# raguilar011095/planet_heightmap_generation

Measured on AMD Instinct MI355X. Metric: Mcells·iter/s, terrain-post erosion stack, higher is better.
Workload: dtype f64

## Files before the change

### planet_heightmap_generation_amd/csrc/device.h

```cpp
#pragma once
#include <hip/hip_runtime.h>

#include <cstdint>
#include <cstdio>
#include <map>
#include <string>
#include <vector>

#include "device_mem.h"
#include "host_util.h"

#include "erode_ops.h"
#include "flood_ops.h"
#include "wo_internal.h"

namespace wo {

#define WO_TRY try {
#define WO_CATCH(fn)                                                                                   \
    } catch (const ::wo::HipError& e) { ::wo::set_error(std::string(fn) + ": " + e.msg); return 2; }   \
      catch (const std::exception& e) { ::wo::set_error(std::string(fn) + ": " + e.what()); return 3; }

constexpr int WO_BLOCK = 256;
inline int blocks_for(int64_t n, int maxBlocks = 1 << 20) {
// ... 82 lines not shown
    wo::FloodExchange floodX;
    void* floodLink = nullptr; void (*floodLinkFree)(void*) = nullptr;
    wo_flood_gpu fgpu;

    int32_t *d_off = nullptr, *d_adj = nullptr;
    float *d_dist = nullptr, *d_xyz = nullptr;
    float *d_e = nullptr, *d_e2 = nullptr, *d_hot = nullptr, *d_orig = nullptr;
    uint8_t *d_ocean = nullptr, *d_coast = nullptr;
    int64_t mirrorMaskVersion = -1;
    uint8_t* d_oceanKnown = nullptr; int32_t* d_maskDiff = nullptr; bool oceanKnownValid = false;
    bool hot_valid = false;
    float* d_savedE = nullptr; uint8_t* d_savedOcean = nullptr; bool saved = false;
    uint8_t* d_tables = nullptr;
    bool scratch = false;
    bool landIdentity = false;
    int64_t floodPrefixMirror = -1, floodPrefixStatic = -1;
    bool floodPrefixOk = false;
    int32_t *d_landIdx = nullptr, *d_land[2] = {nullptr, nullptr}, *d_rank = nullptr;
    int32_t* d_landInit = nullptr; int64_t oceanVersion = 0, landListsOcean = -1; bool landListsMirror = false; int32_t landListsL = -1;
    uint32_t* d_keys[2] = {nullptr, nullptr};
    float *d_cellDist = nullptr, *d_flow = nullptr;
    wo::SolveTask* d_task = nullptr; wo::SolveOut* d_out = nullptr;
    int32_t *d_haloSend = nullptr, *d_haloRecv = nullptr; float *d_haloBuf = nullptr, *h_haloBuf = nullptr; int32_t nHaloSend = 0, nHaloRecv = 0;
    int32_t* d_flowCnt = nullptr; wo::TargetRank* d_tr = nullptr; wo::EventList* d_ev = nullptr; float* d_me = nullptr;
    int32_t *d_carveSlot = nullptr, *d_carveDeps = nullptr, *d_carveDepCnt = nullptr, *d_carveDepPos = nullptr;
    uint32_t* d_rs[2] = {nullptr, nullptr}; int rsFlip[2] = {0, 0};
    wo::CarveRec* d_carveRecs = nullptr; wo::CarveExpect* d_carveExpect = nullptr; unsigned long long* d_carveG = nullptr;
    int32_t* d_carveSlotDone = nullptr; int64_t carveCap = 0;
    unsigned long long* d_accCnt = nullptr;
    int32_t *d_ftLr = nullptr, *d_ftParent = nullptr, *d_ftExtCnt = nullptr; uint32_t* d_ftInflow = nullptr; unsigned long long* d_ftRootAcc = nullptr;
    int32_t *d_jump = nullptr, *d_nj = nullptr;
    int32_t* d_doneAt = nullptr;
    double* d_totalExcess = nullptr;
    float *d_glac = nullptr, *d_iceFlow = nullptr;
    int32_t *d_iceTarget = nullptr, *d_arank = nullptr;
    uint8_t* d_iceUp = nullptr;
    int32_t *d_patchOrder = nullptr, *d_slotOf = nullptr, *d_patchPending = nullptr, *d_patchTotals = nullptr, *d_patchBlk = nullptr;
    int64_t patchVersion = -1; bool patchMirror = false; int32_t numPatches = 0; int64_t lastPatchLaunches = 1; int64_t solveCalls = 0;
    hipStream_t side = nullptr; hipEvent_t evFork = nullptr, evJoin = nullptr; bool onSide = false;
    uint32_t* d_basinKey = nullptr; int32_t* d_basinVals[2] = {nullptr, nullptr}; int32_t *d_basinJ = nullptr, *d_basinSlot = nullptr, *d_basinRange = nullptr;
    uint8_t* d_basinLong = nullptr; int64_t basinLaunches = 0;
    wo::Affine* d_affine[2] = {nullptr, nullptr};
    int64_t solvePassSerial = 0;
    int32_t* h_patchTotals = nullptr;
    int32_t *d_listA = nullptr, *d_listB = nullptr, *d_counters = nullptr;
    void* d_sortTemp = nullptr; size_t sortTempBytes = 0;
    int landCur = 0;
    int32_t L = 0;

    struct Import {
        wo::DeviceArena mem;
        uint8_t* img = nullptr; int64_t imgCap = 0;
        int32_t* label = nullptr;
        uint8_t* flags = nullptr;
        int32_t* lists = nullptr;
        uint8_t* seedOcean = nullptr;
        int32_t* blockCounts = nullptr;
        int32_t* totals = nullptr; int32_t* h_totals = nullptr;
    } imp;

    struct wo_wind_block* wind = nullptr;
    struct wo_ocean_block* ocean = nullptr;
    struct wo_precip_block* precip = nullptr;
    struct wo_temp_block* temp = nullptr;
    struct wo_koppen_block* koppen = nullptr;
    struct wo_map_block* map = nullptr;
// ... 91 lines not shown
```

### planet_heightmap_generation_amd/csrc/erode_ops.h

```cpp
#pragma once
#include <cmath>
#include <cstdint>
#include <cstring>

#include "noise.h"

namespace wo {

constexpr int WO_MAX_DEG = 24;
constexpr int32_t WO_NOT_DONE = 0x7fffffff;

#ifndef WO_TASK_ALIGN
#define WO_TASK_ALIGN 16
#endif
struct alignas(WO_TASK_ALIGN) SolveTask {
    int32_t predSelf, predT, predT2;
    uint32_t flags;
    float e0r, e0t, e0t2;
    float cellDistT;
    double factor;
    int32_t pad_[2];
};
static_assert(sizeof(SolveTask) == 48, "one 48-byte record per task");
#ifndef WO_PATCH_CELLS
// ... 18 lines not shown
    const int32_t* off;
    const int32_t* adj;
    const float* dist;
    const float* xyz;
    const uint8_t* ocean;
    const uint8_t* coast;
    float* e;
    float* e2;
    float* me;
    int32_t L;
    int32_t* land;
    const int32_t* landIdx;
    int32_t xcdTileL;
    int32_t* rank;
    int32_t* target;
    TargetRank* tr;
    float* cellDist;
    float* flow;
    uint32_t* accA; uint32_t* accB;
    unsigned long long* accCnt;
    int32_t* jumpA; int32_t* jumpB;
    SolveTask* task;
    const int32_t* slotOf;
    SolveOut* out;
    double solveK, solveM, solveDt;
    int32_t solveFinals;
    int32_t solveLean;
    int32_t* basinJ;
    const int32_t* basinMslot;
    int32_t* blk;
    EventList* ev;
    int32_t* doneAt;
    double* totalExcess;
    float* glac;
    int32_t* iceTarget;
    float* iceFlow;
    uint8_t* iceUp;
    int32_t* arank;
    const int32_t* carveSlot;
    int32_t* carveDeps;
    int32_t* carveDepCnt;
    int32_t* carveDepPos;
    int32_t* blocker;
};

WO_HD inline double nd_or_eps(float d) { return (d == 0.0f || d != d) ? 1e-6 : (double)d; }

constexpr int WO_ROW = 8;
struct alignas(4) RowI4 { int32_t v[4]; };
struct alignas(4) RowF4 { float v[4]; };
WO_HD inline int load_row(const Fields& F, int32_t r, int32_t& b, int32_t (&nb)[WO_ROW]) {
    b = F.off[r];
    const int deg = F.off[r + 1] - b;
#if defined(__HIP_DEVICE_COMPILE__)
    static_assert(WO_ROW == 8, "two RowI4 per row");
    const RowI4 lo = *reinterpret_cast<const RowI4*>(F.adj + b), hi = *reinterpret_cast<const RowI4*>(F.adj + b + 4);
#pragma unroll
    for (int k = 0; k < 4; ++k) { nb[k] = (k < deg) ? lo.v[k] : r; nb[k + 4] = (k + 4 < deg) ? hi.v[k] : r; }
#else
#pragma unroll
    for (int k = 0; k < WO_ROW; ++k) nb[k] = (k < deg) ? F.adj[b + k] : r;
#endif
    return deg;
}
WO_HD inline void load_row_dist(const Fields& F, int32_t b, int deg, float (&dd)[WO_ROW]) {
#if defined(__HIP_DEVICE_COMPILE__)
// ... 476 lines not shown
#pragma unroll
        for (int k = 0; k < WO_ROW; ++k) if (k < deg && q[k].target == x && q[k].rank < bestRank) { best = nbs[k]; bestRank = q[k].rank; }
    } else {
        for (int32_t j = b; j < b + deg; ++j) {
            const int32_t n = F.adj[j];
            const TargetRank v = F.tr[n];
            if (v.target != x) continue;
            if (v.rank < bestRank) { best = n; bestRank = v.rank; }
        }
    }
    return best;
}
WO_HD inline float solve_final_cell(const Fields& F, int32_t x) {
    if (F.ocean[x]) return F.e[x];
    if (F.ev) {
        const EventList E = F.ev[x];
        if (E.rank[0] != -2) {
            int32_t last = -1;
#pragma unroll
            for (int q = 0; q < WO_EVENTS; ++q) if (E.rank[q] >= 0) last = E.cell[q];
            if (last < 0) return F.e[x];
            return (last == x) ? F.out[store_index(F, x)].self.v : F.out[store_index(F, last)].dep.v;
        }
    }
    const int32_t best = latest_event_cell(F, x);
    if (best < 0) return F.e[x];
    return (best == x) ? F.out[store_index(F, x)].self.v : F.out[store_index(F, best)].dep.v;
}

WO_HD inline float masked_elev_cell(const Fields& F, int32_t r) { return F.ocean[r] ? INFINITY : F.e[r]; }

WO_HD inline bool talus_may_exceed(double x, double d, double talus) { return x > talus * d * (1.0 - 1e-12); }

template <class Masked>
WO_HD inline void thermal_excess_cell_t(const Fields& F, int32_t r, double talus, Masked masked) {
    double total = 0;
    if (!F.ocean[r]) {
        const double h = masked(r);
        int32_t b, nbs[WO_ROW];
        const int deg = load_row(F, r, b, nbs);
        if (deg <= WO_ROW) {
            float mh[WO_ROW], dd[WO_ROW];
#pragma unroll
            for (int k = 0; k < WO_ROW; ++k) mh[k] = masked(nbs[k]);
            load_row_dist(F, b, deg, dd);
#pragma unroll
            for (int k = 0; k < WO_ROW; ++k) {
                const double nh = mh[k];
                if (k >= deg || nh >= h) continue;
                const double d = nd_or_eps(dd[k]);
                if (!talus_may_exceed(h - nh, d, talus)) continue;
                const double slope = (h - nh) / d;
                if (slope > talus) total += (slope - talus) * d;
            }
        } else {
            for (int32_t j = b; j < b + deg; ++j) {
                const double nh = masked(F.adj[j]);
                if (nh >= h) continue;
                const double d = nd_or_eps(F.dist[j]);
                const double slope = (h - nh) / d;
                if (slope > talus) total += (slope - talus) * d;
            }
        }
    }
    F.totalExcess[r] = total;
}

WO_HD inline void thermal_excess_cell(const Fields& F, int32_t r, double talus) { thermal_excess_cell_t(F, r, talus, [&](int32_t c) { return F.me[c]; }); }

template <class Masked>
WO_HD inline float thermal_apply_row(const Fields& F, double h, int32_t myRank, double myTotal, int32_t b, const int32_t (&nbs)[WO_ROW], int deg,
                                     double talus, double kThermal, Masked masked) {
    float mh[WO_ROW], dd[WO_ROW];
#pragma unroll
    for (int k = 0; k < WO_ROW; ++k) mh[k] = masked(nbs[k]);
    load_row_dist(F, b, deg, dd);
    double inSh[WO_ROW], outSh[WO_ROW]; int32_t inRk[WO_ROW]; bool outOn[WO_ROW];
    bool hasOut = false, hasIn = false;
#pragma unroll
    for (int k = 0; k < WO_ROW; ++k) {
        inRk[k] = 0x7fffffff; inSh[k] = 0; outSh[k] = 0; outOn[k] = false;
        const double nh = mh[k], d = nd_or_eps(dd[k]);
        const double gap = fabs(nh - h);
        if (!(k < deg && nh != (double)INFINITY && talus_may_exceed(gap, d, talus))) continue;
        const double slope = gap / d;
        if (!(slope > talus)) continue;
        const bool sends = nh < h;
        if (!sends && !(nh > h)) continue;
// ... 65 lines not shown
    if (nIn == 0 && !hasOut) return (float)(h + 0.0);
    float delta = 0.0f;
    int32_t last = -1;
    for (int phase = 0; phase < 2; ++phase) {
        for (;;) {
            int pick = -1; int32_t pr = 0x7fffffff;
            for (int k = 0; k < nIn; ++k) { const int32_t rk = inRank[k * stride]; if (rk > last && rk < pr) { pr = rk; pick = k; } }
            if (pick < 0 || (phase == 0 && pr > myRank)) break;
            delta = (float)((double)delta + inShare[pick * stride]);
            last = pr;
        }
        if (phase == 0 && hasOut && outShare) {
            for (int k = 0; k < nOut; ++k) delta = (float)((double)delta - outShare[k * stride]);
        } else if (phase == 0 && hasOut) {
            for (int32_t j = b; j < b + deg; ++j) {
                const double nh = (double)F.me[F.adj[j]];
                if (!(nh < h)) continue;
                const double d = nd_or_eps(F.dist[j]);
                const double slope = (h - nh) / d;
                if (slope > talus) {
                    const float excess = (float)((slope - talus) * d);
                    delta = (float)((double)delta - ((double)excess / myTotal) * myTransfer);
                }
            }
        }
    }
    return (float)(h + (double)delta);
}

WO_HD inline float thermal_apply_cell(const Fields& F, int32_t c, double talus, double kThermal, double* inShare, int32_t* inRank, int stride,
                                      double* outShare = nullptr) {
    return thermal_apply_cell_t(F, c, talus, kThermal, inShare, inRank, stride, outShare, [&](int32_t x) { return F.me[x]; });
}

WO_HD inline double smoothstep_js(double x, double e0, double e1) {
    double t = (x - e0) / (e1 - e0);
    if (!(t < 1)) t = (t != t) ? t : 1;
    if (!(t > 0)) t = (t != t) ? t : 0;
    return t * t * (3 - 2 * t);
}

WO_HD inline float glac_index_cell(const Fields& F, int32_t r, double glacialStrength) {
    if (F.ocean[r]) return 0.0f;
    const double PI_ = 3.141592653589793;
    const double thresholdLat = PI_ / 2 - glacialStrength * PI_ / 4.5;
    double y = F.xyz[3 * r + 1];
    if (y > 1) y = 1;
    if (y < -1) y = -1;
    const double polarDist = fabs(asin(y));
    const double latFactor = smoothstep_js(polarDist, thresholdLat, PI_ / 2);
    const double elevFactor = smoothstep_js(F.e[r], 0.5, 0.9);
    const double latScale = smoothstep_js(polarDist, PI_ / 8, PI_ / 3);
    const double a = latFactor, b = elevFactor * 0.3 * (0.3 + 0.7 * latScale);
    return (float)((a > b ? a : b) * glacialStrength);
}

WO_HD inline void ice_receiver_cell(const Fields& F, int32_t r) {
    int32_t bestNb = -1;
    if (!F.ocean[r] && F.glac[r] > 0) {
        const double h = F.e[r];
        double bestDrop = 0;
        for (int32_t j = F.off[r]; j < F.off[r + 1]; ++j) {
            const int32_t nb = F.adj[j];
            const double drop = h - (double)F.e[nb];
            if (drop > bestDrop) { bestDrop = drop; bestNb = nb; }
        }
// ... 243 lines not shown
```

### planet_heightmap_generation_amd/csrc/kernels_impl.h

```cpp
#pragma once
#include <hip/hip_runtime.h>
#include <hip/hip_cooperative_groups.h>

#include "device.h"
#include "plates_ops.h"
#include "climate_ops.h"

namespace wo {

#define WO_GRID_STRIDE(i, n) for (int32_t i = blockIdx.x * blockDim.x + threadIdx.x; i < (n); i += gridDim.x * blockDim.x)

#define WO_XCD_CELLS(r, n)                                                                                           \
    for (int32_t xi_ = (int32_t)(blockIdx.x >> 3), xt_ = F.xcdTile,                                                  \
                 r = (int32_t)((((xi_ / xt_) * 8 + (int32_t)(blockIdx.x & 7u)) * xt_ + (xi_ % xt_)) * (int32_t)blockDim.x + (int32_t)threadIdx.x), \
                 once_ = 1;                                                                                          \
         once_ && r < (n); once_ = 0)

#define WO_XCD_LAND(i, r)                                                                                            \
    for (int32_t xi_ = (int32_t)(blockIdx.x >> 3), xt_ = F.xcdTileL,                                                 \
                 i = (int32_t)((((xi_ / xt_) * 8 + (int32_t)(blockIdx.x & 7u)) * xt_ + (xi_ % xt_)) * (int32_t)blockDim.x + (int32_t)threadIdx.x), \
                 once_ = 1;                                                                                          \
         once_ && i < F.L; once_ = 0)                                                                                \
        for (int32_t r = F.landIdx ? F.landIdx[i] : i, once2_ = 1; once2_; once2_ = 0)

// ... 127 lines not shown
        F.jumpA[r] = -1; F.flow[r] = 0.0f; F.totalExcess[r] = 0.0; F.me[r] = INFINITY;
    }
}
constexpr int WO_TILE_WIN = 4096;
constexpr int WO_TILE_MARGIN = 256;
struct TileWindow {
    const float* g; const float* s; int32_t lo, hi;
    __device__ inline float operator()(int32_t c) const { return (c >= lo && c <= hi) ? s[c - lo] : g[c]; }
};
__device__ inline TileWindow stage_tile(const Fields& F, const float* field, float* s_buf, int32_t i0) {
    TileWindow W; W.g = field; W.s = s_buf; W.lo = 1; W.hi = 0;
    if (!F.tileLds) return W;
    if (i0 < F.L) {
        const int32_t i1 = min(i0 + (int32_t)blockDim.x, F.L) - 1;
        const int32_t lo = max((F.landIdx ? F.landIdx[i0] : i0) - WO_TILE_MARGIN, 0), hi = min((F.landIdx ? F.landIdx[i1] : i1) + WO_TILE_MARGIN, F.N - 1);
        if (hi - lo + 1 <= WO_TILE_WIN) {
            for (int32_t k = threadIdx.x; k <= hi - lo; k += blockDim.x) s_buf[k] = field[lo + k];
            W.lo = lo; W.hi = hi;
        }
    }
    __syncthreads();
    return W;
}
#define WO_XCD_LAND_BASE() ((int32_t)(((((int32_t)(blockIdx.x >> 3) / F.xcdTileL) * 8 + (int32_t)(blockIdx.x & 7u)) * F.xcdTileL + ((int32_t)(blockIdx.x >> 3) % F.xcdTileL)) * (int32_t)blockDim.x))

__global__ __launch_bounds__(WO_BLOCK) void k_receivers_flow_init(Fields F, int32_t* donorCnt) {
    __shared__ float s_tile[WO_TILE_WIN];
    const TileWindow E = stage_tile(F, F.e, s_tile, WO_XCD_LAND_BASE());
    WO_XCD_LAND(i, r) {
        const int32_t t = receiver_cell_t(F, r, E);
        int32_t j = -1; const uint32_t a = 1;
        if (t >= 0 && !F.ocean[t] && F.rank[r] < F.rank[t]) j = t;
        if (F.accA) F.accA[r] = a;
        F.jumpA[r] = j; F.accCnt[r] = 1ull;
        if (j >= 0 && donorCnt) atomicAdd(&donorCnt[j], 1);
        if (F.basinJ) {
            const bool landT = t >= 0 && !F.ocean[t];
            const int32_t sr = F.basinMslot ? F.basinMslot[r] : r;
            F.basinJ[sr] = landT ? (F.basinMslot ? F.basinMslot[t] : t) : sr;
        }
    }
}
__global__ __launch_bounds__(WO_BLOCK) void k_flow_climb(Fields F, const int32_t* donorCnt, int32_t cap) {
    WO_XCD_LAND(i, r) {
        int32_t d = r;
        if (!(donorCnt[d] == 0 && F.jumpA[d] >= 0)) continue;
        unsigned long long v = 1;
        int32_t j = F.jumpA[d];
        for (int32_t step = 0; step < cap; ++step) {
            const int32_t donors = donorCnt[j];
            const int32_t jj = F.jumpA[j];
            const unsigned long long old = atomicAdd(&F.accCnt[j], (1ull << 32) | v);
            F.jumpA[d] = -2;
            if ((int32_t)(old >> 32) + 1 != donors) break;
            if (jj < 0) break;
            d = j;
            j = jj;
            v = (old & 0xffffffffull) + v;
        }
    }
}
#ifndef WO_FT_CELLS
#define WO_FT_CELLS 1024
#endif
#ifndef WO_FT_THREADS
#define WO_FT_THREADS 256
#endif
constexpr int FT_CELLS = WO_FT_CELLS, FT_THREADS = WO_FT_THREADS, FT_PER = FT_CELLS / FT_THREADS;
static_assert(FT_CELLS % FT_THREADS == 0 && FT_CELLS < 0xffff, "tile cells are 16-bit indices");
struct FlowTiles {
    int32_t* lr;
    unsigned long long* rootAcc;
    uint32_t* inflow;
    int32_t* extCnt;
    int32_t* parent;
    int32_t* basinJ;
};
template <bool FINAL>
__global__ __launch_bounds__(FT_THREADS) void k_flow_tiles(Fields F, FlowTiles T) {
    __shared__ uint32_t s_pc[FT_CELLS];
    __shared__ unsigned long long s_acc[FT_CELLS];
    __shared__ uint16_t s_lr[FINAL ? 1 : FT_CELLS];
    __shared__ uint16_t s_b[FINAL ? 1 : FT_CELLS];
    __shared__ int32_t s_bext[FINAL ? 1 : FT_CELLS];
    const int tid = threadIdx.x;
    const int32_t base = (int32_t)blockIdx.x * FT_CELLS;
    const int32_t n = min((int32_t)FT_CELLS, F.L - base);
#pragma unroll
    for (int q = 0; q < FT_PER; ++q) {
        const int i = tid + q * FT_THREADS;
        if (i >= n) continue;
        const int32_t j = F.jumpA[base + i];
        const bool local = j >= base && j < base + n;
        s_pc[i] = local ? (uint32_t)(j - base) : 0xffffu;
        uint32_t w = 1u;
        if (FINAL) { w += T.inflow[base + i]; T.inflow[base + i] = 0u; T.extCnt[base + i] = 0; }
        s_acc[i] = (unsigned long long)w;
        if (!FINAL) s_lr[i] = local ? (uint16_t)(j - base) : (uint16_t)i;
        if (!FINAL && T.basinJ) {
            const int32_t jb = T.basinJ[base + i];
            s_b[i] = (jb >= base && jb < base + n) ? (uint16_t)(jb - base) : (uint16_t)i;
            s_bext[i] = jb;
        }
    }
    __syncthreads();
#pragma unroll
    for (int q = 0; q < FT_PER; ++q) {
        const int i = tid + q * FT_THREADS;
        if (i >= n) continue;
        const uint32_t p = s_pc[i] & 0xffffu;
        if (p != 0xffffu) atomicAdd(&s_pc[p], 1u << 16);
    }
    __syncthreads();
#pragma unroll
    for (int q = 0; q < FT_PER; ++q) {
        const int i = tid + q * FT_THREADS;
        if (i >= n) continue;
        const uint32_t pc0 = s_pc[i];
        if ((pc0 >> 16) != 0u || (pc0 & 0xffffu) == 0xffffu) continue;
        uint32_t p = pc0 & 0xffffu;
        uint32_t v = (uint32_t)s_acc[i];
        for (;;) {
            const uint32_t pcp = s_pc[p];
            const unsigned long long old = atomicAdd(&s_acc[p], (1ull << 32) | (unsigned long long)v);
            if ((uint32_t)(old >> 32) + 1u != (pcp >> 16)) break;
            v += (uint32_t)old;
            p = pcp & 0xffffu;
            if (p == 0xffffu) break;
        }
    }
    __syncthreads();
#pragma unroll
    for (int q = 0; q < FT_PER; ++q) {
        const int i = tid + q * FT_THREADS;
        if (i >= n) continue;
        const uint32_t total = (uint32_t)s_acc[i];
        if (FINAL) F.accCnt[base + i] = (unsigned long long)total;
        else {
            uint16_t r = s_lr[i];
            for (int it = 0; it < FT_CELLS; ++it) {
                const uint16_t rr = s_lr[r];
                if (rr == r) break;
                s_lr[i] = rr;
                r = rr;
            }
            T.lr[base + i] = base + (int32_t)r;
            if ((s_pc[i] & 0xffffu) == 0xffffu) T.rootAcc[base + i] = (unsigned long long)total;
            if (T.basinJ) {
                const uint16_t b0 = s_b[r];
                int32_t out = s_bext[r];
                if (b0 != r) {
                    int32_t res = -1;
                    uint16_t c = b0;
                    for (int it = 0; it < 64; ++it) {
                        const uint16_t cc = s_b[c];
                        if (cc == c) { res = s_bext[c]; break; }
                        if (cc == r) break;
                        c = cc;
                    }
                    out = res >= 0 ? res : ((uint16_t)i == r ? s_bext[i] : base + (int32_t)r);
                }
                T.basinJ[base + i] = out;
            }
        }
    }
}
__global__ __launch_bounds__(WO_BLOCK) void k_flow_root_links(Fields F, FlowTiles T) {
    WO_GRID_STRIDE(i, F.L) {
        if (T.lr[i] != i) continue;
        const int32_t x = F.jumpA[i];
        int32_t P = -1;
        if (x >= 0) { P = T.lr[x]; atomicAdd(&T.extCnt[P], 1); }
        T.parent[i] = P;
    }
}
__global__ __launch_bounds__(WO_BLOCK) void k_flow_root_climb(Fields F, FlowTiles T) {
    WO_GRID_STRIDE(i, F.L) {
        if (T.lr[i] != i || T.extCnt[i] != 0) continue;
        int32_t P = T.parent[i];
        if (P < 0) continue;
        int32_t x = F.jumpA[i];
        uint32_t v = (uint32_t)T.rootAcc[i];
        for (;;) {
            const int32_t need = T.extCnt[P];
            const int32_t PP = T.parent[P];
            const int32_t xx = F.jumpA[P];
            atomicAdd(&T.inflow[x], v);
            const unsigned long long old = atomicAdd(&T.rootAcc[P], (1ull << 32) | (unsigned long long)v);
            if ((int32_t)(old >> 32) + 1 != need) break;
            if (PP < 0) break;
            v += (uint32_t)old;
            P = PP; x = xx;
        }
    }
}

// ... 263 lines not shown
}

__global__ __launch_bounds__(WO_BLOCK) void k_solve_blk_init(Fields F, int32_t L) {
    WO_GRID_STRIDE(s, L) {
        if (F.out[s].self.tag != 0) continue;
        const SolveTask T = F.task[s];
        F.blk[s] = T.predT >= 0 ? T.predT : (T.predSelf >= 0 ? T.predSelf : T.predT2);
    }
}
__global__ __launch_bounds__(WO_BLOCK) void k_slot_scatter(const int32_t* patchOrder, int32_t* slotOf, int32_t L) {
    WO_GRID_STRIDE(s, L) slotOf[patchOrder[s]] = s;
}


__global__ __launch_bounds__(WO_BLOCK) void k_solve_final(Fields F, float* out, float* masked) {
    WO_XCD_LAND(i, r) {
        const float v = solve_final_cell(F, r);
        out[r] = v;
        if (masked) masked[r] = v;
    }
}
__global__ __launch_bounds__(WO_BLOCK) void k_fill_i32(int32_t* a, int32_t v, int32_t n) { WO_GRID_STRIDE(i, n) a[i] = v; }

__global__ __launch_bounds__(WO_BLOCK) void k_masked_elev(Fields F) { WO_XCD_LAND(i, r) F.me[r] = F.e[r]; }
__global__ __launch_bounds__(WO_BLOCK) void k_thermal_excess(Fields F, double talus) {
    __shared__ float s_tile[WO_TILE_WIN];
    const TileWindow M = stage_tile(F, F.me, s_tile, WO_XCD_LAND_BASE());
    WO_XCD_LAND(i, r) thermal_excess_cell_t(F, r, talus, M);
}
#ifndef WO_THERMAL_WAVES
#define WO_THERMAL_WAVES 6
#endif
template <int MAXIN>
__global__ __launch_bounds__(WO_BLOCK, WO_THERMAL_WAVES) void k_thermal_apply_reg(Fields F, float* out, double talus, double kThermal) {
    __shared__ float s_tile[WO_TILE_WIN];
    const TileWindow M = stage_tile(F, F.me, s_tile, WO_XCD_LAND_BASE());
    WO_XCD_LAND(i, r) {
        double inShare[MAXIN], outShare[MAXIN]; int32_t inRank[MAXIN];
        out[r] = thermal_apply_cell_t(F, r, talus, kThermal, inShare, inRank, 1, outShare, M);
    }
}
__global__ __launch_bounds__(WO_BLOCK) void k_thermal_apply(Fields F, float* out, double talus, double kThermal, int32_t maxDeg) {
    extern __shared__ __attribute__((aligned(16))) char smem[];
    double* inShare = reinterpret_cast<double*>(smem) + threadIdx.x;
    int32_t* inRank = reinterpret_cast<int32_t*>(smem + (size_t)maxDeg * WO_BLOCK * sizeof(double)) + threadIdx.x;
    WO_XCD_LAND(i, r) out[r] = thermal_apply_cell(F, r, talus, kThermal, inShare, inRank, WO_BLOCK);
}

__global__ __launch_bounds__(WO_BLOCK) void k_glac_index(Fields F, double strength) { WO_XCD_CELLS(r, F.N) F.glac[r] = glac_index_cell(F, r, strength); }
__global__ __launch_bounds__(WO_BLOCK) void k_ice_receivers(Fields F) {
    WO_XCD_CELLS(r, F.N) { ice_receiver_cell(F, r); F.blocker[r] = 0; if (F.ocean[r]) { F.iceFlow[r] = 0.0f; F.iceUp[r] = 0; } }
}
__device__ inline float ld_agent(const float* p) { return __hip_atomic_load(p, __ATOMIC_RELAXED, __HIP_MEMORY_SCOPE_AGENT); }
__device__ inline int32_t ld_agent(const int32_t* p) { return __hip_atomic_load(p, __ATOMIC_RELAXED, __HIP_MEMORY_SCOPE_AGENT); }
__device__ inline void st_agent(float* p, float v) { __hip_atomic_store(p, v, __ATOMIC_RELAXED, __HIP_MEMORY_SCOPE_AGENT); }
__device__ inline void st_agent(int32_t* p, int32_t v) { __hip_atomic_store(p, v, __ATOMIC_RELAXED, __HIP_MEMORY_SCOPE_AGENT); }
__device__ inline void drain_stores() { asm volatile("s_waitcnt vmcnt(0)" ::: "memory"); }

struct IceRow { int32_t nb[WO_ROW]; int32_t rank[WO_ROW]; uint32_t donors; int nd; int deg; };
__device__ inline void ice_row_of(const Fields& F, int32_t t, IceRow& D) {
    int32_t b;
    D.deg = load_row(F, t, b, D.nb);
    D.donors = 0; D.nd = 0;
    if (D.deg > WO_ROW) {
        for (int32_t j = b; j < b + D.deg; ++j) if (F.iceTarget[F.adj[j]] == t) ++D.nd;
        return;
    }
    int32_t tg[WO_ROW];
#pragma unroll
    for (int k = 0; k < WO_ROW; ++k) { tg[k] = F.iceTarget[D.nb[k]]; D.rank[k] = F.rank[D.nb[k]]; }
#pragma unroll
    for (int k = 0; k < WO_ROW; ++k) if (k < D.deg && tg[k] == t) { D.donors |= 1u << k; ++D.nd; }
}
__device__ inline float ice_task_long_row(const Fields& F, int32_t t, int& up) {
    int32_t dn[WO_MAX_DEG]; int nd = 0;
    for (int32_t j = F.off[t]; j < F.off[t + 1]; ++j) { const int32_t n = F.adj[j]; if (F.iceTarget[n] == t) dn[nd++] = n; }
    float acc = F.glac[t];
    int32_t last = -1;
    up = 0;
// ... 287 lines not shown
```

### planet_heightmap_generation_amd/csrc/planet.hip

```cpp
#include <hip/hip_runtime.h>

#include <algorithm>
#include <atomic>
#include <chrono>
#include <cmath>
#include <cstring>

#include "../../include/worogen.h"
#include "device.h"
#include "elevation_host.h"
#include "elevation_kernels.h"
#include "kernels_impl.h"
#include "flood_kernels.h"
#include "elevation_bfs.h"
#include "noise.h"

namespace wo {

const char* const kFamilyNames[FAM_COUNT] = {
    "coast_flags", "smooth_elevation", "sharpen_ridges", "soil_creep", "warp_terrain", "noise_eval", "synthetic_terrain",
    "ocean_from_elevation", "sort_keys", "sort_radix", "rank_scatter", "receivers", "flow_climb",
    "flow_final", "solve_setup", "solve_round", "solve_final", "thermal_excess", "thermal_apply",
    "glac_index", "ice_receivers", "ice_round", "carve_setup", "carve_round", "moraine_fjord", "glacial_blend", "solve_patch", "elev_collisions", "elev_uplift_fused", "plate_grid", "plate_project", "smooth_field", "flood_eval", "flood_apply", "flood_misc", "climate_sweeps", "basin_layout", "basin_sort", "solve_basin", "flow_tiles", "misc", "event_pair_empty", "event_pair_noop_kernel", "event_pair_two_noop_kernels",
    "map_lonlat", "map_fill", "map_sides", "map_big_boxes", "map_resolve", "map_region_colors", "map_pixels"};

hipEvent_t profile_event(wo_planet* p) {
    if (!p->eventPool.empty()) { hipEvent_t e = p->eventPool.back(); p->eventPool.pop_back(); return e; }
    hipEvent_t e; WO_HIP(hipEventCreate(&e)); return e;
}
void profile_resolve(wo_planet* p) {
    if (p->pending.empty()) return;
    WO_HIP(hipStreamSynchronize(p->ctx->stream));
    if (p->side) WO_HIP(hipStreamSynchronize(p->side));
    for (auto& pe : p->pending) {
        float ms = 0; WO_HIP(hipEventElapsedTime(&ms, pe.a, pe.b));
        p->famMs[pe.fam] += ms; p->famLaunches[pe.fam] += 1;
        p->eventPool.push_back(pe.a); p->eventPool.push_back(pe.b);
    }
    p->pending.clear();
}

constexpr int WO_PATCH_TOTAL_SLOTS = 4096;


static void ensure_scratch(wo_planet* p) {
    if (p->scratch) return;
    const size_t N = (size_t)p->N;
    DeviceArena a;
    p->d_landIdx = a.dev<int32_t>(N); p->d_land[0] = a.dev<int32_t>(N); p->d_land[1] = a.dev<int32_t>(N);
    p->d_keys[0] = a.dev<uint32_t>(N); p->d_keys[1] = a.dev<uint32_t>(N);
    p->d_rank = a.dev<int32_t>(N);
    p->d_cellDist = a.dev<float>(N); p->d_flow = a.dev<float>(N); p->d_task = a.dev<SolveTask>(N);
    p->d_out = a.dev<SolveOut>(N); WO_HIP(hipMemset(p->d_out, 0, N * sizeof(SolveOut)));
    p->d_flowCnt = a.dev<int32_t>(N); WO_HIP(hipMemset(p->d_flowCnt, 0, (size_t)N * 4));
    p->d_tr = a.dev<TargetRank>(N); p->d_ev = a.dev<EventList>(N); p->d_me = a.dev<float>(N); p->d_carveSlot = a.dev<int32_t>(N);
    p->d_accCnt = a.dev<unsigned long long>(N); p->d_jump = a.dev<int32_t>(N); p->d_nj = a.dev<int32_t>(N);
    p->d_doneAt = a.dev<int32_t>(N);
    p->d_totalExcess = a.dev<double>(N);
    p->d_glac = a.dev<float>(N); p->d_iceFlow = a.dev<float>(N); p->d_iceTarget = a.dev<int32_t>(N); p->d_arank = a.dev<int32_t>(N);
    p->d_iceUp = a.dev<uint8_t>(N);
    p->d_listA = a.dev<int32_t>(N); p->d_listB = a.dev<int32_t>(N); p->d_counters = a.dev<int32_t>(8);
    p->d_patchOrder = a.dev<int32_t>(N); p->d_slotOf = a.dev<int32_t>(N); p->d_patchPending = a.dev<int32_t>(N / WO_PATCH + 2);
    p->d_patchTotals = a.dev<int32_t>(WO_PATCH_TOTAL_SLOTS); p->d_patchBlk = a.dev<int32_t>(N);
    p->h_patchTotals = a.pinned<int32_t>(WO_PATCH_TOTAL_SLOTS);
    p->sortTempBytes = sort_temp_bytes(p->N);
    p->d_sortTemp = a.dev<uint8_t>(std::max<size_t>(p->sortTempBytes, 16));
    WO_HIP(hipMemsetAsync(p->d_glac, 0, N * sizeof(float), p->ctx->stream));
    p->mem.adopt(a);
    p->scratch = true;
}

}

wo::Fields wo_planet::fields() const {
    wo::Fields F{};
    F.N = N; F.xcdTile = wo::xcd_tile(N); F.tileLds = opt.tileLds ? 1 : 0; F.off = d_off; F.adj = d_adj; F.dist = d_dist; F.xyz = d_xyz; F.ocean = d_ocean; F.coast = d_coast;
    F.e = d_e; F.e2 = d_e2; F.L = L; F.land = d_land[landCur]; F.landIdx = landIdentity ? nullptr : d_landIdx; F.xcdTileL = wo::xcd_tile(L > 0 ? L : 1); F.rank = d_rank; F.target = nullptr; F.tr = d_tr; F.ev = d_ev; F.me = d_me; F.carveSlot = d_carveSlot; F.carveDeps = nullptr; F.carveDepCnt = d_carveDepCnt; F.carveDepPos = d_carveDepPos; F.cellDist = d_cellDist;
    F.flow = d_flow; F.accA = nullptr; F.accB = nullptr; F.accCnt = d_accCnt; F.jumpA = d_jump; F.jumpB = nullptr;
    F.task = d_task; F.out = d_out; F.slotOf = (patchVersion >= 0) ? d_slotOf : nullptr; F.blk = d_patchBlk; F.doneAt = d_doneAt;
    F.totalExcess = d_totalExcess; F.glac = d_glac; F.iceTarget = d_iceTarget; F.iceFlow = d_iceFlow; F.iceUp = d_iceUp; F.arank = d_arank; F.blocker = d_nj;
    return F;
}

namespace wo {

static inline void swap_elev(wo_planet* p) { std::swap(p->d_e, p->d_e2); }
static inline void ocean_changed(wo_planet* p) { p->h_ocean_valid = false; }
__global__ __launch_bounds__(wo::WO_BLOCK) void k_mask_differs(const uint8_t* __restrict__ a, const uint8_t* __restrict__ b, int32_t N, int32_t* flag) {
    bool diff = false;
    for (int32_t r = blockIdx.x * blockDim.x + threadIdx.x; r < N; r += gridDim.x * blockDim.x) diff |= a[r] != b[r];
    if (diff) atomicOr(flag, 1);
}
static int32_t read_count(wo_planet* p, const int32_t* d_ptr);
static void refresh_host_ocean(wo_planet* p) {
    if (p->h_ocean_valid) return;
    hipStream_t s = p->ctx->stream;
    if (p->d_oceanKnown && p->oceanKnownValid && p->h_ocean.size() == (size_t)p->N) {
        WO_HIP(hipMemsetAsync(p->d_maskDiff, 0, sizeof(int32_t), s));
        hipLaunchKernelGGL(k_mask_differs, dim3(wo::blocks_for(p->N, 1 << 15)), dim3(wo::WO_BLOCK), 0, s, (const uint8_t*)p->d_ocean, (const uint8_t*)p->d_oceanKnown, p->N, p->d_maskDiff);
        if (read_count(p, p->d_maskDiff) == 0) { p->h_ocean_valid = true; return; }
    }
    hvec<uint8_t> tmp(p->N);
    WO_HIP(hipMemcpyAsync(tmp.data(), p->d_ocean, p->N, hipMemcpyDeviceToHost, s));
    WO_HIP(hipStreamSynchronize(s));
    if (tmp.size() != p->h_ocean.size() || std::memcmp(tmp.data(), p->h_ocean.data(), tmp.size()) != 0) {
        p->h_ocean.swap(tmp);
        p->flood.staticValid = false; ++p->oceanVersion;
    }
    p->h_ocean_valid = true;
    if (!p->d_maskDiff) p->d_maskDiff = p->mem.dev<int32_t>(1);
    if (!p->d_oceanKnown) p->d_oceanKnown = p->mem.dev<uint8_t>(p->N);
    WO_HIP(hipMemcpyAsync(p->d_oceanKnown, p->d_ocean, (size_t)p->N, hipMemcpyDeviceToDevice, s));
    p->oceanKnownValid = true;
// ... 594 lines not shown
static void glacial_step_exact(ErodeCall& c) {
    wo_planet* p = c.p;
    c.clk.begin("glacial");
    Fields F = p->fields();
    ice_flow(c, F);
    launch(p, FAM_CARVE_SETUP, k_carve_setup_cells, c.gridN, WO_BLOCK, F);
    select_active_by_rank(p, F.arank, p->d_listB, p->d_counters + 3);
    const int32_t active = read_count(p, p->d_counters + 3);
    c.carveActive += active; ensure_carve_capacity(p, active);
    F.carveDeps = p->d_carveDeps; F.carveDepCnt = p->d_carveDepCnt; F.carveDepPos = p->d_carveDepPos;
    if (active > 0) c.carveRounds += carve_launches(c, F, active);
    launch(p, FAM_MORAINE, k_moraine_fjord, c.gridN, WO_BLOCK, F, c.gDep, c.gFjord);
    c.clk.end();
}
static FlowTiles flow_tiles_buffers(wo_planet* p) {
    const size_t N = (size_t)p->N;
    if (!p->d_ftLr) {
        DeviceArena& a = p->mem;
        if (!p->d_ftParent) p->d_ftParent = a.dev<int32_t>(N);
        if (!p->d_ftExtCnt) p->d_ftExtCnt = a.dev<int32_t>(N);
        if (!p->d_ftInflow) p->d_ftInflow = a.dev<uint32_t>(N);
        if (!p->d_ftRootAcc) p->d_ftRootAcc = a.dev<unsigned long long>(N);
        p->d_ftLr = a.dev<int32_t>(N);
        WO_HIP(hipMemsetAsync(p->d_ftInflow, 0, N * 4, p->ctx->stream)); WO_HIP(hipMemsetAsync(p->d_ftExtCnt, 0, N * 4, p->ctx->stream));
    }
    FlowTiles FT{};
    FT.lr = p->d_ftLr; FT.parent = p->d_ftParent; FT.rootAcc = p->d_ftRootAcc; FT.inflow = p->d_ftInflow; FT.extCnt = p->d_ftExtCnt;
    return FT;
}
static int flow_tile_count(int32_t L) { return (int)(((int64_t)L + FT_CELLS - 1) / FT_CELLS); }
static void erode_receivers(ErodeCall& c, const Fields& F, const FlowTiles& FT, int32_t* donorCnt, bool basin, bool slotIdentity, bool tilesBeforeFork) {
    wo_planet* p = c.p; hipStream_t s = p->ctx->stream;
    Fields Fr = F; if (basin) Fr.basinJ = p->d_basinJ;
    c.clk.begin("receivers");
    launch(p, FAM_RECEIVERS, k_receivers_flow_init, c.gridL, WO_BLOCK, Fr, donorCnt);
    c.clk.end();
    if (!basin) return;
    ensure_side_stream(p);
    if (tilesBeforeFork) {
        launch(p, FAM_FLOW_TILES, k_flow_tiles<false>, flow_tile_count(p->L), FT_THREADS, F, FT);
        launch(p, FAM_FLOW_TILES, k_flow_root_links, blocks_for(p->L, 4096), WO_BLOCK, F, FT);
    }
    WO_HIP(hipEventRecord(p->evFork, s));
    WO_HIP(hipStreamWaitEvent(p->side, p->evFork, 0));
    p->onSide = true;
    try { basin_layout(p, slotIdentity); } catch (...) { p->onSide = false; throw; }
    p->onSide = false;
    WO_HIP(hipEventRecord(p->evJoin, p->side));
}
static void erode_flow(ErodeCall& c, const Fields& F, const FlowTiles& FT, int32_t* donorCnt, bool flowTiles, bool tilesBeforeFork, bool clearOut) {
    wo_planet* p = c.p;
    c.clk.begin("flow");
    if (flowTiles) {
        const int tiles = flow_tile_count(p->L);
        if (!tilesBeforeFork) {
            launch(p, FAM_FLOW_TILES, k_flow_tiles<false>, tiles, FT_THREADS, F, FT);
            launch(p, FAM_FLOW_TILES, k_flow_root_links, blocks_for(p->L, 4096), WO_BLOCK, F, FT);
        }
        launch(p, FAM_FLOW_TILES, k_flow_root_climb, blocks_for(p->L, 4096), WO_BLOCK, F, FT);
        launch(p, FAM_FLOW_TILES, k_flow_tiles<true>, tiles, FT_THREADS, F, FT);
    } else
        launch(p, FAM_FLOW_SNAP, k_flow_climb, c.gridL, WO_BLOCK, F, (const int32_t*)p->d_flowCnt, (int32_t)0x7fffffff);
    Fields Ff = F;
    if (p->opt.relaxedFull) Ff.ev = nullptr;
    launch(p, FAM_FLOW_FINAL, k_flow_final, c.gridL, WO_BLOCK, Ff, donorCnt, clearOut ? p->d_out : (SolveOut*)nullptr);
    c.clk.end();
// ... 18 lines not shown
    wo_planet* p = c.p;
    if (!p->d_affine[1]) p->d_affine[1] = p->mem.dev<Affine>((size_t)p->N);
    if (!p->d_affine[0]) p->d_affine[0] = p->mem.dev<Affine>((size_t)p->N);
    launch(p, FAM_SOLVE_SETUP, k_affine_init, c.gridL, WO_BLOCK, F, p->d_affine[0]);
    int cur = 0;
    for (int q = 0; q < 12; ++q, cur ^= 1) launch(p, FAM_SOLVE_ROUND, k_affine_jump, c.gridL, WO_BLOCK, F, (const Affine*)p->d_affine[cur], p->d_affine[cur ^ 1]);
    launch(p, FAM_SOLVE_FINAL, k_affine_apply, c.gridL, WO_BLOCK, F, (const Affine*)p->d_affine[cur], p->d_e2);
}
static void hydraulic_step(ErodeCall& c, int32_t iter) {
    wo_planet* p = c.p;
    Fields F = p->fields();
    F.solveK = c.K; F.solveM = c.m; F.solveDt = c.dt;
    const bool basin = !p->opt.relaxedFull;
    const bool slotIdentity = c.mir.on && p->mirror.h_mask.size() == (size_t)p->N;
    if (basin) { basin_alloc(p); F.basinMslot = slotIdentity ? nullptr : p->d_slotOf; }
    const bool flowTiles = p->landIdentity;
    FlowTiles FT = flowTiles ? flow_tiles_buffers(p) : FlowTiles{};
    const bool tilesBeforeFork = basin && flowTiles && slotIdentity;
    if (tilesBeforeFork) FT.basinJ = p->d_basinJ;
    int32_t* const donorCnt = flowTiles ? (int32_t*)nullptr : p->d_flowCnt;
    erode_receivers(c, F, FT, donorCnt, basin, slotIdentity, tilesBeforeFork);
    erode_flow(c, F, FT, donorCnt, flowTiles, tilesBeforeFork, basin && c.checkEveryPass);
    c.clk.begin("solve");
    if (basin) erode_solve_basin(c, F, iter); else erode_solve_affine(c, F);
    swap_elev(p);
    c.clk.end();
}
static void thermal_step(ErodeCall& c, bool afterSolve) {
    wo_planet* p = c.p;
    c.clk.begin("thermal");
    const Fields F = p->fields();
    if (!afterSolve) launch(p, FAM_THERMAL_EXCESS, k_masked_elev, c.gridL, WO_BLOCK, F);
    launch(p, FAM_THERMAL_EXCESS, k_thermal_excess, c.gridL, WO_BLOCK, F, c.talus);
    if (p->maxDeg <= 12) launch(p, FAM_THERMAL_APPLY, k_thermal_apply_reg<12>, c.gridL, WO_BLOCK, F, p->d_e2, c.talus, c.kThermal);
    else if (p->maxDeg <= 16) launch(p, FAM_THERMAL_APPLY, k_thermal_apply_reg<16>, c.gridL, WO_BLOCK, F, p->d_e2, c.talus, c.kThermal);
    else launch_shmem(p, FAM_THERMAL_APPLY, k_thermal_apply, c.gridL, WO_BLOCK, (size_t)p->maxDeg * WO_BLOCK * 12, F, p->d_e2, c.talus, c.kThermal, (int32_t)p->maxDeg);
    swap_elev(p);
    c.clk.end();
}

static void erode_composite(wo_planet* p, int32_t hIters, double K, double m, double dt, int32_t tIters, double talus,
                            double kThermal, int32_t gIters, double gStrength, bool checkEveryPass = true) {
    ErodeCall c(p, hIters, K, m, dt, tIters, talus, kThermal, gIters, gStrength, checkEveryPass);
    release_stage_brackets(p);
    p->stageTiming.clear(); p->erodeStats.clear();
    p->floodX.calls = 0; p->floodX.gathers = 0; p->floodX.globalFloods = 0; p->floodX.received = 0;
    if (c.total <= 0) return;
    ensure_scratch(p);
    hipStream_t s = p->ctx->stream;
    if (hIters > 0) WO_HIP(hipMemsetAsync(p->d_flowCnt, 0, (size_t)p->N * sizeof(int32_t), s));
    if (hIters > 0 && p->d_ftInflow) { WO_HIP(hipMemsetAsync(p->d_ftInflow, 0, (size_t)p->N * 4, s)); WO_HIP(hipMemsetAsync(p->d_ftExtCnt, 0, (size_t)p->N * 4, s)); }
    if (!erode_setup(c)) return;
    if (hIters > 0) erode_flood(c, 0.5);

    const bool glacial = c.gIters > 0 && c.gStrength > 0;
    if (glacial) launch(p, FAM_GLAC_INDEX, k_glac_index, c.gridN, WO_BLOCK, p->fields(), c.gStrength);
    const bool relaxedFull = p->opt.relaxedFull;
    bool midDone = false, sortAfterFlood = false;
    for (int32_t iter = 0; iter < c.total; ++iter) {
        c.clk.on = true;
        if (!midDone && iter >= c.midIter) { midDone = true; erode_flood(c, 0.85); sortAfterFlood = true; }
        c.clk.on = p->opt.stageTimingAll || p->profiling || c.total <= 16 || iter % 8 == 0;
        const bool gNow = iter < c.gIters && glacial, hNow = iter < hIters;
        const bool sortNow = relaxedFull ? (iter == 0 || sortAfterFlood) : (p->opt.relaxedSortEvery <= 1 || iter % p->opt.relaxedSortEvery == 0);
        if ((gNow || hNow) && sortNow) { sortAfterFlood = false; erode_sort(c); }
        if (gNow) { if (relaxedFull) glacial_step_relaxed(c); else glacial_step_exact(c); }
        if (hNow) {
            if (gNow && sortNow) erode_sort(c);
            hydraulic_step(c, iter);
        }
// ... 931 lines not shown
```

Before: 6265.

## Skip thermal apply for inactive cells and update elevation in place

The thermal excess pass now marks each land cell as "hot" when any neighbour gap could exceed talus. The apply kernel then writes into e in place only for hot cells, which drops the double-buffer swap and the full output write. The non-final flow-tile kernel also replaces the per-tile accumulation pass with a plain root-count via shared atomics, and the accCnt init store is skipped when unused. The risk is correctness: in-place updates rely on cold cells producing no change, and the new root accumulation semantics must match the old ones.

```diff
diff --git a/planet_heightmap_generation_amd/csrc/device.h b/planet_heightmap_generation_amd/csrc/device.h
--- a/planet_heightmap_generation_amd/csrc/device.h
+++ b/planet_heightmap_generation_amd/csrc/device.h
@@ -138,6 +138,7 @@
     int32_t *d_jump = nullptr, *d_nj = nullptr;
     int32_t* d_doneAt = nullptr;
     double* d_totalExcess = nullptr;
+    uint8_t* d_thermalHot = nullptr;
     float *d_glac = nullptr, *d_iceFlow = nullptr;
     int32_t *d_iceTarget = nullptr, *d_arank = nullptr;
     uint8_t* d_iceUp = nullptr;
diff --git a/planet_heightmap_generation_amd/csrc/erode_ops.h b/planet_heightmap_generation_amd/csrc/erode_ops.h
--- a/planet_heightmap_generation_amd/csrc/erode_ops.h
+++ b/planet_heightmap_generation_amd/csrc/erode_ops.h
@@ -74,6 +74,7 @@
     EventList* ev;
     int32_t* doneAt;
     double* totalExcess;
+    uint8_t* thermalHot;
     float* glac;
     int32_t* iceTarget;
     float* iceFlow;
@@ -616,11 +617,14 @@
 
 WO_HD inline bool talus_may_exceed(double x, double d, double talus) { return x > talus * d * (1.0 - 1e-12); }
 
+WO_HD inline bool thermal_hot_value(float h) { uint32_t u; std::memcpy(&u, &h, 4); return h != h || u == 0x80000000u; }
+
 template <class Masked>
 WO_HD inline void thermal_excess_cell_t(const Fields& F, int32_t r, double talus, Masked masked) {
     double total = 0;
     if (!F.ocean[r]) {
-        const double h = masked(r);
+        const float hf = masked(r);
+        const double h = hf;
         int32_t b, nbs[WO_ROW];
         const int deg = load_row(F, r, b, nbs);
         if (deg <= WO_ROW) {
@@ -628,16 +632,21 @@
 #pragma unroll
             for (int k = 0; k < WO_ROW; ++k) mh[k] = masked(nbs[k]);
             load_row_dist(F, b, deg, dd);
+            bool hot = thermal_hot_value(hf);
 #pragma unroll
             for (int k = 0; k < WO_ROW; ++k) {
                 const double nh = mh[k];
-                if (k >= deg || nh >= h) continue;
                 const double d = nd_or_eps(dd[k]);
-                if (!talus_may_exceed(h - nh, d, talus)) continue;
-                const double slope = (h - nh) / d;
+                const double gap = h - nh;
+                const bool may = k < deg && talus_may_exceed(fabs(gap), d, talus);
+                hot = hot || (may && mh[k] != INFINITY);
+                if (!may || !(nh < h)) continue;
+                const double slope = gap / d;
                 if (slope > talus) total += (slope - talus) * d;
             }
+            if (F.thermalHot) F.thermalHot[r] = hot ? 1 : 0;
         } else {
+            if (F.thermalHot) F.thermalHot[r] = 1;
             for (int32_t j = b; j < b + deg; ++j) {
                 const double nh = masked(F.adj[j]);
                 if (nh >= h) continue;
@@ -769,6 +778,16 @@
                                       double* outShare = nullptr) {
     return thermal_apply_cell_t(F, c, talus, kThermal, inShare, inRank, stride, outShare, [&](int32_t x) { return F.me[x]; });
 }
+template <class Masked>
+WO_HD inline void thermal_apply_hot_cell_t(const Fields& F, int32_t c, double talus, double kThermal, double* inShare, int32_t* inRank, int stride,
+                                           double* outShare, Masked masked) {
+    if (!F.thermalHot[c]) return;
+    F.e[c] = thermal_apply_cell_t(F, c, talus, kThermal, inShare, inRank, stride, outShare, masked);
+}
+WO_HD inline void thermal_apply_hot_cell(const Fields& F, int32_t c, double talus, double kThermal, double* inShare, int32_t* inRank, int stride,
+                                         double* outShare = nullptr) {
+    thermal_apply_hot_cell_t(F, c, talus, kThermal, inShare, inRank, stride, outShare, [&](int32_t x) { return F.me[x]; });
+}
 
 WO_HD inline double smoothstep_js(double x, double e0, double e1) {
     double t = (x - e0) / (e1 - e0);
diff --git a/planet_heightmap_generation_amd/csrc/kernels_impl.h b/planet_heightmap_generation_amd/csrc/kernels_impl.h
--- a/planet_heightmap_generation_amd/csrc/kernels_impl.h
+++ b/planet_heightmap_generation_amd/csrc/kernels_impl.h
@@ -183,7 +183,8 @@
         int32_t j = -1; const uint32_t a = 1;
         if (t >= 0 && !F.ocean[t] && F.rank[r] < F.rank[t]) j = t;
         if (F.accA) F.accA[r] = a;
-        F.jumpA[r] = j; F.accCnt[r] = 1ull;
+        F.jumpA[r] = j;
+        if (F.accCnt) F.accCnt[r] = 1ull;
         if (j >= 0 && donorCnt) atomicAdd(&donorCnt[j], 1);
         if (F.basinJ) {
             const bool landT = t >= 0 && !F.ocean[t];
@@ -230,7 +231,8 @@
 template <bool FINAL>
 __global__ __launch_bounds__(FT_THREADS) void k_flow_tiles(Fields F, FlowTiles T) {
     __shared__ uint32_t s_pc[FT_CELLS];
-    __shared__ unsigned long long s_acc[FT_CELLS];
+    __shared__ unsigned long long s_acc[FINAL ? FT_CELLS : 1];
+    __shared__ uint32_t s_cnt[FINAL ? 1 : FT_CELLS];
     __shared__ uint16_t s_lr[FINAL ? 1 : FT_CELLS];
     __shared__ uint16_t s_b[FINAL ? 1 : FT_CELLS];
     __shared__ int32_t s_bext[FINAL ? 1 : FT_CELLS];
@@ -244,50 +246,59 @@
         const int32_t j = F.jumpA[base + i];
         const bool local = j >= base && j < base + n;
         s_pc[i] = local ? (uint32_t)(j - base) : 0xffffu;
-        uint32_t w = 1u;
-        if (FINAL) { w += T.inflow[base + i]; T.inflow[base + i] = 0u; T.extCnt[base + i] = 0; }
-        s_acc[i] = (unsigned long long)w;
-        if (!FINAL) s_lr[i] = local ? (uint16_t)(j - base) : (uint16_t)i;
-        if (!FINAL && T.basinJ) {
-            const int32_t jb = T.basinJ[base + i];
-            s_b[i] = (jb >= base && jb < base + n) ? (uint16_t)(jb - base) : (uint16_t)i;
-            s_bext[i] = jb;
+        if constexpr (FINAL) {
+            const uint32_t w = 1u + T.inflow[base + i];
+            T.inflow[base + i] = 0u; T.extCnt[base + i] = 0;
+            s_acc[i] = (unsigned long long)w;
+        } else {
+            s_cnt[i] = 0u;
+            s_lr[i] = local ? (uint16_t)(j - base) : (uint16_t)i;
+            if (T.basinJ) {
+                const int32_t jb = T.basinJ[base + i];
+                s_b[i] = (jb >= base && jb < base + n) ? (uint16_t)(jb - base) : (uint16_t)i;
+                s_bext[i] = jb;
+            }
         }
     }
     __syncthreads();
-#pragma unroll
-    for (int q = 0; q < FT_PER; ++q) {
-        const int i = tid + q * FT_THREADS;
-        if (i >= n) continue;
-        const uint32_t p = s_pc[i] & 0xffffu;
-        if (p != 0xffffu) atomicAdd(&s_pc[p], 1u << 16);
-    }
-    __syncthreads();
-#pragma unroll
-    for (int q = 0; q < FT_PER; ++q) {
-        const int i = tid + q * FT_THREADS;
-        if (i >= n) continue;
-        const uint32_t pc0 = s_pc[i];
-        if ((pc0 >> 16) != 0u || (pc0 & 0xffffu) == 0xffffu) continue;
-        uint32_t p = pc0 & 0xffffu;
-        uint32_t v = (uint32_t)s_acc[i];
-        for (;;) {
-            const uint32_t pcp = s_pc[p];
-            const unsigned long long old = atomicAdd(&s_acc[p], (1ull << 32) | (unsigned long long)v);
-            if ((uint32_t)(old >> 32) + 1u != (pcp >> 16)) break;
-            v += (uint32_t)old;
-            p = pcp & 0xffffu;
-            if (p == 0xffffu) break;
-        }
-    }
-    __syncthreads();
-#pragma unroll
-    for (int q = 0; q < FT_PER; ++q) {
-        const int i = tid + q * FT_THREADS;
-        if (i >= n) continue;
-        const uint32_t total = (uint32_t)s_acc[i];
-        if (FINAL) F.accCnt[base + i] = (unsigned long long)total;
-        else {
+    if constexpr (FINAL) {
+#pragma unroll
+        for (int q = 0; q < FT_PER; ++q) {
+            const int i = tid + q * FT_THREADS;
+            if (i >= n) continue;
+            const uint32_t p = s_pc[i] & 0xffffu;
+            if (p != 0xffffu) atomicAdd(&s_pc[p], 1u << 16);
+        }
+        __syncthreads();
+#pragma unroll
+        for (int q = 0; q < FT_PER; ++q) {
+            const int i = tid + q * FT_THREADS;
+            if (i >= n) continue;
+            const uint32_t pc0 = s_pc[i];
+            if ((pc0 >> 16) != 0u || (pc0 & 0xffffu) == 0xffffu) continue;
+            uint32_t p = pc0 & 0xffffu;
+            uint32_t v = (uint32_t)s_acc[i];
+            for (;;) {
+                const uint32_t pcp = s_pc[p];
+                const unsigned long long old = atomicAdd(&s_acc[p], (1ull << 32) | (unsigned long long)v);
+                if ((uint32_t)(old >> 32) + 1u != (pcp >> 16)) break;
+                v += (uint32_t)old;
+                p = pcp & 0xffffu;
+                if (p == 0xffffu) break;
+            }
+        }
+        __syncthreads();
+#pragma unroll
+        for (int q = 0; q < FT_PER; ++q) {
+            const int i = tid + q * FT_THREADS;
+            if (i >= n) continue;
+            F.accCnt[base + i] = (unsigned long long)(uint32_t)s_acc[i];
+        }
+    } else {
+#pragma unroll
+        for (int q = 0; q < FT_PER; ++q) {
+            const int i = tid + q * FT_THREADS;
+            if (i >= n) continue;
             uint16_t r = s_lr[i];
             for (int it = 0; it < FT_CELLS; ++it) {
                 const uint16_t rr = s_lr[r];
@@ -295,8 +306,8 @@
                 s_lr[i] = rr;
                 r = rr;
             }
+            atomicAdd(&s_cnt[r], 1u);
             T.lr[base + i] = base + (int32_t)r;
-            if ((s_pc[i] & 0xffffu) == 0xffffu) T.rootAcc[base + i] = (unsigned long long)total;
             if (T.basinJ) {
                 const uint16_t b0 = s_b[r];
                 int32_t out = s_bext[r];
@@ -313,6 +324,12 @@
                 }
                 T.basinJ[base + i] = out;
             }
+        }
+        __syncthreads();
+#pragma unroll
+        for (int q = 0; q < FT_PER; ++q) {
+            const int i = tid + q * FT_THREADS;
+            if (i < n && (s_pc[i] & 0xffffu) == 0xffffu) T.rootAcc[base + i] = (unsigned long long)s_cnt[i];
         }
     }
 }
@@ -642,19 +659,19 @@
 #define WO_THERMAL_WAVES 6
 #endif
 template <int MAXIN>
-__global__ __launch_bounds__(WO_BLOCK, WO_THERMAL_WAVES) void k_thermal_apply_reg(Fields F, float* out, double talus, double kThermal) {
+__global__ __launch_bounds__(WO_BLOCK, WO_THERMAL_WAVES) void k_thermal_apply_reg(Fields F, double talus, double kThermal) {
     __shared__ float s_tile[WO_TILE_WIN];
     const TileWindow M = stage_tile(F, F.me, s_tile, WO_XCD_LAND_BASE());
     WO_XCD_LAND(i, r) {
         double inShare[MAXIN], outShare[MAXIN]; int32_t inRank[MAXIN];
-        out[r] = thermal_apply_cell_t(F, r, talus, kThermal, inShare, inRank, 1, outShare, M);
-    }
-}
-__global__ __launch_bounds__(WO_BLOCK) void k_thermal_apply(Fields F, float* out, double talus, double kThermal, int32_t maxDeg) {
+        thermal_apply_hot_cell_t(F, r, talus, kThermal, inShare, inRank, 1, outShare, M);
+    }
+}
+__global__ __launch_bounds__(WO_BLOCK) void k_thermal_apply(Fields F, double talus, double kThermal, int32_t maxDeg) {
     extern __shared__ __attribute__((aligned(16))) char smem[];
     double* inShare = reinterpret_cast<double*>(smem) + threadIdx.x;
     int32_t* inRank = reinterpret_cast<int32_t*>(smem + (size_t)maxDeg * WO_BLOCK * sizeof(double)) + threadIdx.x;
-    WO_XCD_LAND(i, r) out[r] = thermal_apply_cell(F, r, talus, kThermal, inShare, inRank, WO_BLOCK);
+    WO_XCD_LAND(i, r) thermal_apply_hot_cell(F, r, talus, kThermal, inShare, inRank, WO_BLOCK);
 }
 
 __global__ __launch_bounds__(WO_BLOCK) void k_glac_index(Fields F, double strength) { WO_XCD_CELLS(r, F.N) F.glac[r] = glac_index_cell(F, r, strength); }
diff --git a/planet_heightmap_generation_amd/csrc/planet.hip b/planet_heightmap_generation_amd/csrc/planet.hip
--- a/planet_heightmap_generation_amd/csrc/planet.hip
+++ b/planet_heightmap_generation_amd/csrc/planet.hip
@@ -56,7 +56,7 @@
     p->d_tr = a.dev<TargetRank>(N); p->d_ev = a.dev<EventList>(N); p->d_me = a.dev<float>(N); p->d_carveSlot = a.dev<int32_t>(N);
     p->d_accCnt = a.dev<unsigned long long>(N); p->d_jump = a.dev<int32_t>(N); p->d_nj = a.dev<int32_t>(N);
     p->d_doneAt = a.dev<int32_t>(N);
-    p->d_totalExcess = a.dev<double>(N);
+    p->d_totalExcess = a.dev<double>(N); p->d_thermalHot = a.dev<uint8_t>(N);
     p->d_glac = a.dev<float>(N); p->d_iceFlow = a.dev<float>(N); p->d_iceTarget = a.dev<int32_t>(N); p->d_arank = a.dev<int32_t>(N);
     p->d_iceUp = a.dev<uint8_t>(N);
     p->d_listA = a.dev<int32_t>(N); p->d_listB = a.dev<int32_t>(N); p->d_counters = a.dev<int32_t>(8);
@@ -78,7 +78,7 @@
     F.e = d_e; F.e2 = d_e2; F.L = L; F.land = d_land[landCur]; F.landIdx = landIdentity ? nullptr : d_landIdx; F.xcdTileL = wo::xcd_tile(L > 0 ? L : 1); F.rank = d_rank; F.target = nullptr; F.tr = d_tr; F.ev = d_ev; F.me = d_me; F.carveSlot = d_carveSlot; F.carveDeps = nullptr; F.carveDepCnt = d_carveDepCnt; F.carveDepPos = d_carveDepPos; F.cellDist = d_cellDist;
     F.flow = d_flow; F.accA = nullptr; F.accB = nullptr; F.accCnt = d_accCnt; F.jumpA = d_jump; F.jumpB = nullptr;
     F.task = d_task; F.out = d_out; F.slotOf = (patchVersion >= 0) ? d_slotOf : nullptr; F.blk = d_patchBlk; F.doneAt = d_doneAt;
-    F.totalExcess = d_totalExcess; F.glac = d_glac; F.iceTarget = d_iceTarget; F.iceFlow = d_iceFlow; F.iceUp = d_iceUp; F.arank = d_arank; F.blocker = d_nj;
+    F.totalExcess = d_totalExcess; F.thermalHot = d_thermalHot; F.glac = d_glac; F.iceTarget = d_iceTarget; F.iceFlow = d_iceFlow; F.iceUp = d_iceUp; F.arank = d_arank; F.blocker = d_nj;
     return F;
 }
 
@@ -739,6 +739,7 @@
 static void erode_receivers(ErodeCall& c, const Fields& F, const FlowTiles& FT, int32_t* donorCnt, bool basin, bool slotIdentity, bool tilesBeforeFork) {
     wo_planet* p = c.p; hipStream_t s = p->ctx->stream;
     Fields Fr = F; if (basin) Fr.basinJ = p->d_basinJ;
+    if (!donorCnt) Fr.accCnt = nullptr;
     c.clk.begin("receivers");
     launch(p, FAM_RECEIVERS, k_receivers_flow_init, c.gridL, WO_BLOCK, Fr, donorCnt);
     c.clk.end();
@@ -823,10 +824,9 @@
     const Fields F = p->fields();
     if (!afterSolve) launch(p, FAM_THERMAL_EXCESS, k_masked_elev, c.gridL, WO_BLOCK, F);
     launch(p, FAM_THERMAL_EXCESS, k_thermal_excess, c.gridL, WO_BLOCK, F, c.talus);
-    if (p->maxDeg <= 12) launch(p, FAM_THERMAL_APPLY, k_thermal_apply_reg<12>, c.gridL, WO_BLOCK, F, p->d_e2, c.talus, c.kThermal);
-    else if (p->maxDeg <= 16) launch(p, FAM_THERMAL_APPLY, k_thermal_apply_reg<16>, c.gridL, WO_BLOCK, F, p->d_e2, c.talus, c.kThermal);
-    else launch_shmem(p, FAM_THERMAL_APPLY, k_thermal_apply, c.gridL, WO_BLOCK, (size_t)p->maxDeg * WO_BLOCK * 12, F, p->d_e2, c.talus, c.kThermal, (int32_t)p->maxDeg);
-    swap_elev(p);
+    if (p->maxDeg <= 12) launch(p, FAM_THERMAL_APPLY, k_thermal_apply_reg<12>, c.gridL, WO_BLOCK, F, c.talus, c.kThermal);
+    else if (p->maxDeg <= 16) launch(p, FAM_THERMAL_APPLY, k_thermal_apply_reg<16>, c.gridL, WO_BLOCK, F, c.talus, c.kThermal);
+    else launch_shmem(p, FAM_THERMAL_APPLY, k_thermal_apply, c.gridL, WO_BLOCK, (size_t)p->maxDeg * WO_BLOCK * 12, F, c.talus, c.kThermal, (int32_t)p->maxDeg);
     c.clk.end();
 }
 
```

New measurement: 6376, median of 6. +1.8%, better.
